# audeering/opensmile

Hardware: AMD Instinct MI355X
Metric: MFCC frames/sec (16kHz, 25ms/10ms) (higher is better)
Workload: dtype f32

## Files before the change

### opensmile_amd/csrc/lld_mfcc512.hip

```cpp
#include <hip/hip_runtime.h>
#include "kernel_timing.hpp"
#include "phase_timing.hpp"
#include "wave_lifetimes.hpp"

#include <algorithm>
#include <cmath>
#include <cstdio>
#include <cstdlib>
#include <cstring>
#include <type_traits>
#include <vector>

#include "lld_device.hpp"
#include "lld_launch.hpp"
#include "lld_params.hpp"
#include "tables.hpp"

namespace smilehip {

namespace {

constexpr int kWavesPerBlock = 8;
constexpr int kTileFrames = 32;
constexpr int kTB2Row = 65;
constexpr int kTB2Floats = 2 * (15 * kTB2Row + 3 * 16 + 16);
constexpr int kLmelFloats = 68;
constexpr int kOctetFloats = 12;
constexpr int kPbFloats = 448;
constexpr int kWaveFloats = 2080;

static_assert(kWaveFloats >= kTB2Floats && kWaveFloats >= 4 * (kLmelFloats + kPbFloats) && kWaveFloats % 4 == 0, "per-wave LDS region");
static_assert(kPbFloats % 64 == 0 && kPbFloats >= 33 * kOctetFloats, "power buffer");
static_assert(kLmelFloats >= 64 && kLmelFloats % 4 == 0 && (kLmelFloats / 4) % 2 == 1,
              "band vectors: room for the PLP vectors at +32 and +48, 16-byte aligned, neighbouring groups on different bank quads");

constexpr float C1 = 0.92387953251128673848f;
constexpr float S1 = 0.38268343236508978178f;
constexpr float R2 = 0.70710678118654752440f;

__device__ __forceinline__ void wave_lds_fence() {
  __builtin_amdgcn_fence(__ATOMIC_ACQ_REL, "wavefront");
  __builtin_amdgcn_wave_barrier();
}

__host__ __device__ constexpr int pb_pos(int k) { return k + (kOctetFloats - 8) * (k >> 3); }

__device__ __forceinline__ void dft4(float &r0, float &i0, float &r1, float &i1, float &r2, float &i2,
                                     float &r3, float &i3) {
  const float t0r = r0 + r2, t0i = i0 + i2;
  const float t1r = r0 - r2, t1i = i0 - i2;
  const float t2r = r1 + r3, t2i = i1 + i3;
  const float t3r = r1 - r3, t3i = i1 - i3;
  r0 = t0r + t2r; i0 = t0i + t2i;
  r2 = t0r - t2r; i2 = t0i - t2i;
  r1 = t1r + t3i; i1 = t1i - t3r;
  r3 = t1r - t3i; i3 = t1i + t3r;
}

__device__ __forceinline__ void cmul(float &r, float &i, float c, float s) {
  const float nr = fmaf(r, c, -i * s);
  const float ni = fmaf(r, s, i * c);
  r = nr; i = ni;
}
__device__ __forceinline__ void cmul_ns(float &r, float &i, float c, float s, float ns) {
  const float nr = fmaf(r, c, i * ns);
  const float ni = fmaf(r, s, i * c);
  r = nr; i = ni;
}

struct Dft16K {
  float c1, s1, r2, nc1, ns1, nr2;
  __device__ __forceinline__ Dft16K() : c1(C1), s1(S1), r2(R2), nc1(-C1), ns1(-S1), nr2(-R2) {
    asm volatile("" : "+s"(c1), "+s"(s1), "+s"(r2), "+s"(nc1), "+s"(ns1), "+s"(nr2));
  }
};

__device__ __forceinline__ void dft16_first(float (&re)[16], float (&im)[16], int m0) {
  dft4(re[m0], im[m0], re[m0 + 4], im[m0 + 4], re[m0 + 8], im[m0 + 8], re[m0 + 12], im[m0 + 12]);
}
__device__ __forceinline__ void dft16_twiddles(float (&re)[16], float (&im)[16], const Dft16K &K) {
  cmul_ns(re[1 + 4], im[1 + 4], K.c1, K.ns1, K.s1);
  { const float a = re[1 + 8], b = im[1 + 8]; re[1 + 8] = K.r2 * (a + b); im[1 + 8] = K.r2 * (b - a); }
  cmul_ns(re[1 + 12], im[1 + 12], K.s1, K.nc1, K.c1);
  { const float a = re[2 + 4], b = im[2 + 4]; re[2 + 4] = K.r2 * (a + b); im[2 + 4] = K.r2 * (b - a); }
  { const float a = re[2 + 8], b = im[2 + 8]; re[2 + 8] = b; im[2 + 8] = -a; }
  { const float a = re[2 + 12], b = im[2 + 12]; re[2 + 12] = K.r2 * (b - a); im[2 + 12] = K.nr2 * (a + b); }
  cmul_ns(re[3 + 4], im[3 + 4], K.s1, K.nc1, K.c1);
  { const float a = re[3 + 8], b = im[3 + 8]; re[3 + 8] = K.r2 * (b - a); im[3 + 8] = K.nr2 * (a + b); }
  cmul_ns(re[3 + 12], im[3 + 12], K.nc1, K.s1, K.ns1);
}
__device__ __forceinline__ void dft16_last(float (&re)[16], float (&im)[16], int q) {
  dft4(re[4 * q], im[4 * q], re[4 * q + 1], im[4 * q + 1], re[4 * q + 2], im[4 * q + 2], re[4 * q + 3], im[4 * q + 3]);
}
__device__ __forceinline__ void dft16_rename(float (&re)[16], float (&im)[16]) {
  float tr[16], ti[16];
#pragma unroll
  for (int q = 0; q < 4; ++q)
#pragma unroll
    for (int p = 0; p < 4; ++p) { tr[q + 4 * p] = re[4 * q + p]; ti[q + 4 * p] = im[4 * q + p]; }
#pragma unroll
  for (int k = 0; k < 16; ++k) { re[k] = tr[k]; im[k] = ti[k]; }
}
__device__ __forceinline__ void dft16(float (&re)[16], float (&im)[16], const Dft16K &K) {
#pragma unroll
  for (int m0 = 0; m0 < 4; ++m0) dft16_first(re, im, m0);
  dft16_twiddles(re, im, K);
#pragma unroll
  for (int q = 0; q < 4; ++q) dft16_last(re, im, q);
  dft16_rename(re, im);
}

template <int CTRL>
__device__ __forceinline__ float dpp_f(float v) {
  return __int_as_float(__builtin_amdgcn_update_dpp(0, __float_as_int(v), CTRL, 0xf, 0xf, true));
}

}

template <int MP, bool PLP, bool DELTA>
constexpr bool typed_loads() {
  return !PLP && !(MP == 16 && DELTA);
}
typedef float float2v __attribute__((ext_vector_type(2)));
__device__ float2v tbuffer_load_xy(__amdgpu_buffer_rsrc_t rsrc, int voffset, int soffset, int format, int aux)
    __asm("llvm.amdgcn.raw.ptr.tbuffer.load.v2f32");
__device__ float tbuffer_load_x(__amdgpu_buffer_rsrc_t rsrc, int voffset, int soffset, int format, int aux)
    __asm("llvm.amdgcn.raw.ptr.tbuffer.load.f32");
constexpr int kFmt16x2Sscaled = 5 | (3 << 4);
constexpr int kFmt16Sscaled = 2 | (3 << 4);
constexpr int kRsrcWord3 = 0x00020000, kRsrcWord3Typed = 0x00020000 | 4 | (5 << 3);

template <int MP, bool ALIGNED, bool TYPED>
struct FrameRegs {
  uint32_t v[ALIGNED && !TYPED ? MP : 2 * MP];
};

template <int MP, bool ALIGNED, bool TYPED>
__device__ __forceinline__ void pcm_prefetch(const int16_t *pcm, int64_t pcm_total, int64_t base, int H, int lane,
                                             FrameRegs<MP, ALIGNED, TYPED> &R) {
  const int64_t b0 = base < 0 ? 0 : base;
  int64_t left = (pcm_total - b0) * 2;
  left = left < 0 ? 0 : (left > 0xfffffffcLL ? 0xfffffffcLL : left);
  const __amdgpu_buffer_rsrc_t rsrc = __builtin_amdgcn_make_buffer_rsrc(const_cast<int16_t *>(pcm + b0), 0, (int)(uint32_t)left,
                                                                        TYPED ? kRsrcWord3Typed : kRsrcWord3);
  uint32_t lo = ((uint32_t)(lane >> 4) * (uint32_t)H + 2u * (uint32_t)(lane & 15)) * 2u + (uint32_t)((base - b0) * 2);
  asm volatile("" : "+v"(lo));
#pragma unroll
  for (int m = 0; m < MP; ++m) {
    if constexpr (TYPED && ALIGNED) {
      const float2v f = tbuffer_load_xy(rsrc, (int)lo + 64 * m, 0, kFmt16x2Sscaled, 0);
      R.v[2 * m] = __float_as_uint(f.x);
      R.v[2 * m + 1] = __float_as_uint(f.y);
    } else if constexpr (TYPED) {
      R.v[2 * m] = __float_as_uint(tbuffer_load_x(rsrc, (int)lo + 64 * m, 0, kFmt16Sscaled, 0));
      R.v[2 * m + 1] = __float_as_uint(tbuffer_load_x(rsrc, (int)lo + 64 * m + 2, 0, kFmt16Sscaled, 0));
    } else if constexpr (ALIGNED) {
      R.v[m] = (uint32_t)__builtin_amdgcn_raw_buffer_load_b32(rsrc, (int)lo + 64 * m, 0, 0);
    } else {
      R.v[2 * m] = (uint32_t)(int32_t)(int16_t)__builtin_amdgcn_raw_buffer_load_b16(rsrc, (int)lo + 64 * m, 0, 0);
      R.v[2 * m + 1] = (uint32_t)(int32_t)(int16_t)__builtin_amdgcn_raw_buffer_load_b16(rsrc, (int)lo + 64 * m + 2, 0, 0);
    }
  }
}

SMILEHIP_PHASE_COUNTERS(g_phase, 16, smilehip_debug_phase)
SMILEHIP_WAVE_LIFE_RECORDS(g_wave_life, smilehip_debug_wave_life)

__device__ __forceinline__ void wave_set_prio(int level) {
  switch (level & 3) {
    case 0: __builtin_amdgcn_s_setprio(0); break;
    case 1: __builtin_amdgcn_s_setprio(1); break;
    case 2: __builtin_amdgcn_s_setprio(2); break;
    default: __builtin_amdgcn_s_setprio(3); break;
  }
}

template <int MP, bool PREEMPH, bool USE_POWER, bool ALIGNED, bool PLP, int UC, bool DELTA, bool PAD0>
__device__ __forceinline__ void lld_mfcc512_body(const LldParams &P, const Fast512Tables &F) {
  extern __shared__ __attribute__((aligned(16))) float smem[];
  const int lane = threadIdx.x & 63;
  const int wave = __builtin_amdgcn_readfirstlane(threadIdx.x >> 6);
  const int g = lane >> 4;
  const int j = lane & 15;

  float2 *s_tw512 = reinterpret_cast<float2 *>(smem);
  float2 *s_win = s_tw512 + 256;
  float2 *s_tw256 = s_win + MP * 16;
  float4 *s_melw0 = reinterpret_cast<float4 *>(s_tw256 + 256);
  float4 *s_melw1 = s_melw0 + UC * 16;
  float *s_dct = reinterpret_cast<float *>(s_melw1 + UC * 16);
  float *s_plp = s_dct + 16 * 28;
  constexpr int shared_floats = 256 * 2 + MP * 16 * 2 + 256 * 2 + UC * 16 * 8 + 16 * 28 + 48;
  float *wbase = smem + shared_floats + wave * kWaveFloats;
  float *s_lmel = wbase + g * kLmelFloats;
  float *s_cep = s_lmel + 48;
  float *s_pb = wbase + 4 * kLmelFloats + g * kPbFloats;

  for (int i = threadIdx.x; i < 256; i += blockDim.x) { s_tw512[i] = F.tw512[i]; s_tw256[i] = F.tw256[i]; }
  for (int i = threadIdx.x; i < MP * 16; i += blockDim.x) s_win[i] = F.win[i];
  for (int i = threadIdx.x; i < UC * 16; i += blockDim.x) { s_melw0[i] = F.melw[2 * i]; s_melw1[i] = F.melw[2 * i + 1]; }
  for (int i = threadIdx.x; i < 16 * 28; i += blockDim.x) s_dct[i] = F.dct28[i];
  if (PLP) {
    for (int i = threadIdx.x; i < 32; i += blockDim.x) s_plp[i] = F.plp_eql[i];
    for (int i = threadIdx.x; i < 16; i += blockDim.x) s_plp[32 + i] = F.plp_sin[i];
  }
  __syncthreads();

  uint32_t mo[UC];
#pragma unroll
  for (int i = 0; i < UC; ++i) mo[i] = F.melo[i * 16 + j];
  const uint32_t lane_bands = (uint32_t)F.lane_bands[j];
  const int band0 = (int)((lane_bands >> 8) & 0xffu), band1 = (int)((lane_bands >> 16) & 0xffu);
  float uf0[UC], uf1[UC];
#pragma unroll
  for (int i = 0; i < UC; ++i) { uf0[i] = ((lane_bands >> i) & 1u) ? 1.0f : 0.0f; uf1[i] = 1.0f - uf0[i]; }
  const uint32_t out_off = (uint32_t)(g * (int)P.ld_out + j) * 4u;
  const uint32_t out_off_d = out_off + (uint32_t)P.n_mfcc * 4u;
  const uint32_t out_off_dd = out_off + (uint32_t)P.n_mfcc * 8u;
  const float nkpre = P.de ? P.k : -P.k;
  const int m0 = P.pad_left >> 5, j0 = (P.pad_left >> 1) & 15;
  float *pb_k = s_pb + pb_pos(j);
  float *pb_m = s_pb + pb_pos(256 - j);

  const Dft16K dk;
  PhaseTimer<12> PH;
  const int tile_stride = __builtin_amdgcn_readfirstlane((int)gridDim.x) * kWavesPerBlock;
  int tile = blockIdx.x * kWavesPerBlock + wave;
  const int n_tiles = DELTA ? P.n_ftiles : P.n_tiles;
  if (tile >= n_tiles) return;
  typedef typename std::conditional<DELTA, FTileRec, TileRec>::type Rec;
  typedef const __attribute__((address_space(4))) Rec *ConstRecPtr;
  const ConstRecPtr recs = DELTA ? (ConstRecPtr)(uintptr_t)P.ftile_rec : (ConstRecPtr)(uintptr_t)P.tile_rec;
  int64_t cur_samp0 = recs[tile].samp0, cur_row0 = recs[tile].row0;
  int cur_n = recs[tile].n_frames;
  int cur_live = 0, cur_e0 = 0, cur_e1 = 0, cur_lo = 0, cur_don = 0;
  if constexpr (DELTA) {
    cur_live = recs[tile].live_n; cur_e0 = recs[tile].e0; cur_e1 = recs[tile].e1; cur_lo = recs[tile].lo; cur_don = recs[tile].delta_on;
  }
  bool has_next = tile + tile_stride < n_tiles;
  int64_t nxt_samp0 = cur_samp0;
  if (has_next) nxt_samp0 = recs[tile + tile_stride].samp0;
  int tp = 0;
  constexpr bool TYPED = typed_loads<MP, PLP, DELTA>();
  FrameRegs<MP, ALIGNED, TYPED> R;
  pcm_prefetch<MP, ALIGNED, TYPED>(P.pcm, P.pcm_total, cur_samp0 - P.pad_left, P.H, lane, R);
  unsigned char *pend_row = nullptr;
  float pend_val = 0.0f;
  bool pend_live = false;
  float s_prev = 0.0f, d_cur = 0.0f;
  int b_tp = 0, b_lo = 0, b_live = 0, b_e0 = 0, b_e1 = 0, b_don = 0;
  const auto from_group = [&](int grp, float v) {
    return __int_as_float(__builtin_amdgcn_ds_bpermute(4 * ((grp << 4) | j), __float_as_int(v)));
  };
  const auto regress = [](float vm2, float vm1, float vp1, float vp2) {
    float num = 0.0f;
    num += 1.0f * (vp1 - vm1);
    num += 2.0f * (vp2 - vm2);
    return num;
  };
  const auto div10 = [](float a, bool &plain) {
    const float y = 0.1f, b = 10.0f;
    plain |= div_needs_division(a);
    return div_markstein(a, b, y);
  };
  const auto delta_fast = [&](float s_cur, float dp, float &dn, float &ddn, float &drow, bool &plain) {
    const float s1 = from_group((g + 1) & 3, g == 0 ? s_cur : s_prev);
    const float s3 = from_group((g + 3) & 3, g == 3 ? s_prev : s_cur);
    dn = div10(regress(s_prev, s1, s3, s_cur), plain);
    const float d1 = from_group((g + 1) & 3, g == 0 ? dn : dp);
    const float d3 = from_group((g + 3) & 3, g == 3 ? dp : dn);
    ddn = div10(regress(dp, d1, d3, dn), plain);
    drow = from_group((g + 2) & 3, g >= 2 ? dp : dn);
  };
  const auto delta_exact = [&](float s_cur, float dp, int btp, int lo, int live_n, float &dn, float &ddn, float &drow) {
    const auto fetch = [&](int x, int hi_c, int base, float cur, float prev) {
      x = x < lo ? lo : (x > hi_c ? hi_c : x);
      const int dd = x - base;
      const float c = from_group(dd & 3, cur), p = from_group(dd & 3, prev);
      return dd >= 0 ? c : p;
    };
    const float norm = 10.0f;
    const int fd = btp - 2 + g, fdd = btp - 4 + g, hi0 = live_n - 1, hi1 = live_n + 1;
    dn = regress(fetch(fd - 2, hi0, btp, s_cur, s_prev), fetch(fd - 1, hi0, btp, s_cur, s_prev), fetch(fd + 1, hi0, btp, s_cur, s_prev),
                 fetch(fd + 2, hi0, btp, s_cur, s_prev)) / norm;
    ddn = regress(fetch(fdd - 2, hi1, btp - 2, dn, dp), fetch(fdd - 1, hi1, btp - 2, dn, dp), fetch(fdd + 1, hi1, btp - 2, dn, dp),
                  fetch(fdd + 2, hi1, btp - 2, dn, dp)) / norm;
    drow = from_group((g + 2) & 3, g >= 2 ? dp : dn);
  };

  const int slot = (int)(__builtin_amdgcn_s_getreg((3 << 11) | 4) & 3u);
  int passes_done = 0;
  WaveLife WL;
  WL.begin();
  for (;;) {
    wave_set_prio(passes_done + slot);
    passes_done += 1;
    const bool live = tp + g < (DELTA ? cur_live : cur_n);
    PH(0);
    if constexpr (!DELTA) {
      if (pend_row != nullptr && pend_live) {
        uint32_t oo = out_off;
        asm volatile("" : "+v"(oo));
        *reinterpret_cast<float *>(pend_row + oo) = pend_val;
      }
    }
    float st_dn = 0.0f, st_ddn = 0.0f, st_drow = 0.0f;
    bool st_plain = false;
    if constexpr (DELTA) delta_fast(pend_val, d_cur, st_dn, st_ddn, st_drow, st_plain);
    float re[16], im[16];
    {
      float tprev = 0.0f;
      (void)tprev;
#pragma unroll
      for (int m = 0; m < 16; ++m) {
        if (m < MP) {
          float a, b;
          if constexpr (TYPED) {
            a = __uint_as_float(R.v[2 * m]);
            b = __uint_as_float(R.v[2 * m + 1]);
          } else if constexpr (ALIGNED) {
            a = (float)(int16_t)(R.v[m] & 0xffffu);
            b = (float)(int16_t)(R.v[m] >> 16);
          } else {
            a = (float)(int32_t)R.v[2 * m];
            b = (float)(int32_t)R.v[2 * m + 1];
          }
          float ya = a, yb = b;
          if (PREEMPH) {
            const float t = dpp_f<0x121>(b);
            const float pa = (j == 0) ? tprev : t;
            tprev = t;
            yb = fmaf(nkpre, a, b);
            ya = fmaf(nkpre, pa, a);
            if (PAD0 ? (m == 0 && j == 0) : (m == m0 && j == j0)) ya = P.one_minus_k * a;
          }
          const float2 w = s_win[m * 16 + j];
          re[m] = ya * w.x;
          im[m] = yb * w.y;
        } else {
          re[m] = 0.0f; im[m] = 0.0f;
        }
      }
    }
    PH(1);
    if constexpr (DELTA) {
      const bool clamped = !(b_tp - 6 >= b_lo && b_tp + 3 <= b_live - 1);
      if (clamped || __builtin_amdgcn_ballot_w64(st_plain && j < P.n_mfcc) != 0) delta_exact(pend_val, d_cur, b_tp, b_lo, b_live, st_dn, st_ddn, st_drow);
      const int fdd = b_tp - 4 + g;
      const bool row_live = pend_row != nullptr && j < P.n_mfcc && fdd >= b_e0 && fdd < b_e1;
      if (row_live) {
        uint32_t oo = out_off;
        asm volatile("" : "+v"(oo));
        *reinterpret_cast<float *>(pend_row + oo) = s_prev;
      }
      if (row_live && b_don) {
        uint32_t oo = out_off_d;
        asm volatile("" : "+v"(oo));
        *reinterpret_cast<float *>(pend_row + oo) = st_drow;
        oo = out_off_dd;
        asm volatile("" : "+v"(oo));
        *reinterpret_cast<float *>(pend_row + oo) = st_ddn;
      }
      s_prev = pend_val;
      d_cur = st_dn;
    }

    float2 *tbw = reinterpret_cast<float2 *>(wbase) + g * 16 + j;
    const float2 *tbr = reinterpret_cast<const float2 *>(wbase) + g * 16 + j * kTB2Row;
    {
      float2 w[4], wn[4];
#pragma unroll
      for (int p = 1; p < 4; ++p) w[p] = s_tw256[(4 * p) * 16 + j];
      w[0] = make_float2(1.0f, 0.0f);
#pragma unroll
      for (int m0 = 0; m0 < 4; ++m0) dft16_first(re, im, m0);
      dft16_twiddles(re, im, dk);
#pragma unroll
      for (int q = 0; q < 4; ++q) {
        if (q < 3) {
#pragma unroll
          for (int p = 0; p < 4; ++p) wn[p] = s_tw256[(q + 1 + 4 * p) * 16 + j];
        }
        dft16_last(re, im, q);
#pragma unroll
        for (int p = 0; p < 4; ++p) {
          const int k1 = q + 4 * p;
          if (k1 > 0) cmul(re[4 * q + p], im[4 * q + p], w[p].x, w[p].y);
          tbw[k1 * kTB2Row] = make_float2(re[4 * q + p], im[4 * q + p]);
        }
#pragma unroll
        for (int p = 0; p < 4; ++p) w[p] = wn[p];
      }
    }
    PH(3);
    {
      wave_lds_fence();
#pragma unroll
      for (int jj = 0; jj < 16; ++jj) {
        typedef const volatile __attribute__((address_space(3))) unsigned long long *LdsU64;
        const unsigned long long v = ((LdsU64)tbr)[jj];
        re[jj] = __int_as_float((int)(uint32_t)v); im[jj] = __int_as_float((int)(uint32_t)(v >> 32));
      }
      wave_lds_fence();
    }
    PH(4);
    dft16(re, im, dk);
    PH(5);

    float zr[8], zi[8];
#pragma unroll
    for (int q = 0; q < 8; ++q) {
      const float pr = q > 0 ? dpp_f<0x12f>(re[(16 - q) & 15]) : re[15];
      const float pi = q > 0 ? dpp_f<0x12f>(im[(16 - q) & 15]) : im[15];
      const float tr = __int_as_float(__builtin_amdgcn_update_dpp(__float_as_int(pr), __float_as_int(re[15 - q]), 0x101, 0xf, 0xf, false));
      const float ti = __int_as_float(__builtin_amdgcn_update_dpp(__float_as_int(pi), __float_as_int(im[15 - q]), 0x101, 0xf, 0xf, false));
      zr[q] = dpp_f<0x140>(tr);
      zi[q] = dpp_f<0x140>(ti);
    }
    float2 tw5[8];
#pragma unroll
    for (int q = 0; q < 8; ++q) tw5[q] = s_tw512[j + 16 * q];
#pragma unroll
    for (int q = 0; q < 8; ++q) {
      const float2 w = tw5[q];
      const float a = re[q], b = im[q];
      const float c = zr[q], d = zi[q];
      const float sr = a + c, si = b - d, dr = a - c, di = b + d;
      const float ur = fmaf(w.x, dr, -w.y * di);
      const float ui = fmaf(w.x, di, w.y * dr);
      const float xr = sr + ui, xi = si - ur;
      const float yr = sr - ui, yi = si + ur;
      float pk = fmaf(xi, xi, xr * xr);
      float pm = fmaf(yi, yi, yr * yr);
      if (q == 0 && j == 0) {
        const float v0 = 2.0f * (a + b), v1 = 2.0f * (a - b);
        pk = v0 * v0; pm = v1 * v1;
      }
      if (!USE_POWER) { pk = sqrtf(pk); pm = sqrtf(pm); }
      pb_k[(2 * kOctetFloats) * q] = pk;
      pb_m[-(2 * kOctetFloats) * q] = pm;
    }
    if (j == 0) {
      const float a = re[8], b = im[8];
      const float s = 4.0f * fmaf(b, b, a * a);
      s_pb[pb_pos(128)] = USE_POWER ? s : sqrtf(s);
    } else if (j < 8) {
      s_pb[pb_pos(256) + j] = 0.0f;
    }
    wave_lds_fence();

    PH(6);
    int ntp = tp + 4;
    const bool advance = ntp >= cur_n;
    const bool more = !advance || has_next;
    if (advance) ntp = 0;
    if (more)
      pcm_prefetch<MP, ALIGNED, TYPED>(P.pcm, P.pcm_total, (advance ? nxt_samp0 : cur_samp0) + (int64_t)ntp * P.H - P.pad_left, P.H, lane, R);
    else if constexpr (TYPED) {
#pragma unroll
      for (int m = 0; m < 2 * MP; ++m) R.v[m] = 0u;
    }

    PH(7);
    {
      float a0 = 0.0f, a1 = 0.0f;
#pragma unroll
      for (int i = 0; i < UC; ++i) {
        const float4 *pp = reinterpret_cast<const float4 *>(reinterpret_cast<const unsigned char *>(s_pb) + mo[i]);
        const float4 p0 = pp[0], p1 = pp[1];
        const float4 w0 = s_melw0[i * 16 + j], w1 = s_melw1[i * 16 + j];
        float acc = p0.x * w0.x;
        acc = fmaf(p0.y, w0.y, acc); acc = fmaf(p0.z, w0.z, acc); acc = fmaf(p0.w, w0.w, acc);
        acc = fmaf(p1.x, w1.x, acc); acc = fmaf(p1.y, w1.y, acc); acc = fmaf(p1.z, w1.z, acc); acc = fmaf(p1.w, w1.w, acc);
        a0 = fmaf(acc, uf0[i], a0);
        a1 = fmaf(acc, uf1[i], a1);
      }
      PH(8);
#pragma unroll
      for (int h = 0; h < 2; ++h) {
        const int b = h ? band1 : band0;
        const float acc = h ? a1 : a0;
        if (b != 0xff) {
          if (PLP) {
            float v = acc * F.mel_scale;
            v = v < P.melfloor ? P.melfloor : v;
            s_lmel[b] = __expf(P.plp_compression * __logf(v * s_plp[b]));
          } else {
            s_lmel[b] = log_mel_fast(acc * F.mel_scale, P.melfloor, P.log_floor);
          }
        }
      }
      if (j + 16 >= P.n_bands) s_lmel[j + 16] = 0.0f;
      if (j >= P.n_bands) s_lmel[j] = 0.0f;
    }
    wave_lds_fence();

    PH(9);
    if (PLP) {
      float *s_acf = s_lmel + 32;
      if (j <= P.plp_order) s_acf[j] = plp_acf_lag(s_lmel, s_dct + j * 28, P.n_bands);
      wave_lds_fence();
      if (j == 0) plp_cc_serial(s_acf, P.plp_order, s_plp + 32, s_cep);
      wave_lds_fence();
      if (j < P.n_mfcc) pend_val = s_cep[j];
    } else
    if (j < P.n_mfcc) {
      const float4 *row_c = reinterpret_cast<const float4 *>(s_dct + j * 28);
      const float4 *lm = reinterpret_cast<const float4 *>(s_lmel);
      float acc = 0.0f, dgain = 0.0f;
#pragma unroll
      for (int q = 0; q < 7; ++q) {
        const float4 l = lm[q], c = row_c[q];
        acc = fmaf(l.x, c.x, acc); acc = fmaf(l.y, c.y, acc); acc = fmaf(l.z, c.z, acc);
        if (q < 6) acc = fmaf(l.w, c.w, acc); else dgain = c.w;
      }
      pend_val = acc * dgain;
    }
    pend_live = live && j < P.n_mfcc;
    pend_row = reinterpret_cast<unsigned char *>(P.out + (cur_row0 + tp - (DELTA ? 4 : 0)) * P.ld_out);
    if constexpr (DELTA) { b_tp = tp; b_lo = cur_lo; b_live = cur_live; b_e0 = cur_e0; b_e1 = cur_e1; b_don = cur_don; }
    wave_lds_fence();
    PH(10);
    if (!more) break;
    if (advance) {
      tile += tile_stride;
      cur_samp0 = nxt_samp0; cur_row0 = recs[tile].row0; cur_n = recs[tile].n_frames;
      if constexpr (DELTA) {
        cur_live = recs[tile].live_n; cur_e0 = recs[tile].e0; cur_e1 = recs[tile].e1; cur_lo = recs[tile].lo; cur_don = recs[tile].delta_on;
      }
      has_next = tile + tile_stride < n_tiles;
      if (has_next) nxt_samp0 = recs[tile + tile_stride].samp0;
    }
    tp = ntp;
  }
  if constexpr (DELTA) {
    float dn, ddn, drow;
    delta_exact(pend_val, d_cur, b_tp, b_lo, b_live, dn, ddn, drow);
    const int fdd = b_tp - 4 + g;
    if (j < P.n_mfcc && fdd >= b_e0 && fdd < b_e1) {
      *reinterpret_cast<float *>(pend_row + out_off) = s_prev;
      if (b_don) {
        *reinterpret_cast<float *>(pend_row + out_off_d) = drow;
        *reinterpret_cast<float *>(pend_row + out_off_dd) = ddn;
      }
    }
  } else if (pend_live) {
    uint32_t oo = out_off;
    asm volatile("" : "+v"(oo));
    *reinterpret_cast<float *>(pend_row + oo) = pend_val;
  }
  PH.flush(g_phase);
  WL.end(g_wave_life, blockIdx.x, (unsigned)wave, (unsigned)passes_done);
}

template <int MP, bool PREEMPH, bool USE_POWER, bool ALIGNED, bool PLP, int UC, bool DELTA = false>
__global__ void __launch_bounds__(kWavesPerBlock * 64, 4) lld_mfcc512(LldParams P, Fast512Tables F) {
  lld_mfcc512_body<MP, PREEMPH, USE_POWER, ALIGNED, PLP, UC, DELTA, true>(P, F);
}
template <int MP, bool PREEMPH, bool USE_POWER, bool ALIGNED, bool PLP, int UC, bool DELTA = false>
__global__ void __launch_bounds__(kWavesPerBlock * 64, 4) lld_mfcc512_padded(LldParams P, Fast512Tables F) {
  lld_mfcc512_body<MP, PREEMPH, USE_POWER, ALIGNED, PLP, UC, DELTA, false>(P, F);
}

bool fast512_applicable(int Nfft, int N) { return Nfft == 512 && N <= 512 && N >= 2; }

int fast512_tile_frames() { return kTileFrames; }

int fast512_build_host(const smilehip_lld_config &cfg, const Geometry &geo, const std::vector<float> &window,
                       const MelBank &mel, const DctTables &dct, Fast512Host &h) {
  const int pad_left = cfg.zero_pad_symmetric ? (int)((geo.Nfft - geo.N) / 2) : 0;
  const int H = (int)geo.H, N = (int)geo.N;
  if (mel.n_bands > 27 || dct.n_mfcc > 16 || cfg.win_offset != 0.0 || (pad_left & 1) || (H & 1) || H < 2) return -1;
  h.mp = (pad_left + N) <= 13 * 32 ? 13 : 16;
  const char *fp = getenv("SMILEHIP_MFCC512_FORCE_PADDED");
  h.force_padded = fp != nullptr && fp[0] == '1';
  h.tw256.resize(256);
  for (int k1 = 0; k1 < 16; ++k1)
    for (int j = 0; j < 16; ++j) {
      const double a = -2.0 * M_PI * double(j * k1) / 256.0;
      h.tw256[k1 * 16 + j] = make_float2(float(cos(a)), float(sin(a)));
    }
  h.tw512.resize(256);
  for (int k = 0; k < 256; ++k) {
    const double a = -2.0 * M_PI * double(k) / 512.0;
    h.tw512[k] = make_float2(float(cos(a)), float(sin(a)));
  }
  h.win.assign(size_t(h.mp) * 16, make_float2(0.f, 0.f));
  for (int m = 0; m < h.mp; ++m)
    for (int j = 0; j < 16; ++j) {
      const int n = 2 * (j + 16 * m) - pad_left;
      float a = 0.f, b = 0.f;
      if (n >= 0 && n < N) a = float(double(window[n]) / 32767.0);
      if (n + 1 >= 0 && n + 1 < N) b = float(double(window[n + 1]) / 32767.0);
      h.win[size_t(m) * 16 + j] = make_float2(a, b);
    }
  struct Unit { int octet; float w[8]; };
  std::vector<Unit> units;
  const int nb = mel.n_bands;
  std::vector<int> first_unit(nb + 1, 0);
  for (int b = 0; b < nb; ++b) {
    int lo = -1, hi = -1;
    if (mel.rise_hi[b] > mel.rise_lo[b]) { lo = mel.rise_lo[b]; hi = mel.rise_hi[b]; }
    if (mel.fall_hi[b] > mel.fall_lo[b]) { if (lo < 0) lo = mel.fall_lo[b]; hi = mel.fall_hi[b]; }
    first_unit[b] = int(units.size());
    if (lo >= 0) {
      for (int o = lo / 8; o <= (hi - 1) / 8; ++o) {
        Unit un;
        un.octet = o;
        for (int e = 0; e < 8; ++e) {
          const int n = 8 * o + e;
          float w = 0.0f;
          if (n >= mel.rise_lo[b] && n < mel.rise_hi[b]) w = 1.0f - mel.coef[n];
          else if (n >= mel.fall_lo[b] && n < mel.fall_hi[b]) w = mel.coef[n];
          un.w[e] = w;
        }
        units.push_back(un);
      }
    }
  }
  first_unit[nb] = int(units.size());
  h.n_slots = int(units.size());
  std::vector<int> size(nb), order(nb);
  for (int b = 0; b < nb; ++b) { size[b] = first_unit[b + 1] - first_unit[b]; order[b] = b; }
  std::stable_sort(order.begin(), order.end(), [&](int x, int y) { return size[x] > size[y]; });
  int cap = 0;
  std::vector<std::pair<int, int>> lanes;
  for (int c : {6, 8}) {
    lanes.clear();
    std::vector<char> used(nb, 0);
    bool ok = true;
    for (int oi = 0; oi < nb && ok; ++oi) {
      const int a = order[oi];
      if (used[a]) continue;
      used[a] = 1;
      if (size[a] > c) { ok = false; break; }
      int partner = -1;
      for (int oj = oi + 1; oj < nb; ++oj)
        if (!used[order[oj]] && size[a] + size[order[oj]] <= c) { partner = order[oj]; break; }
      if (partner >= 0) used[partner] = 1;
      lanes.push_back({a, partner});
    }
    if (ok && (int)lanes.size() <= 16) { cap = c; break; }
  }
  if (cap == 0) return -1;
  h.mel_units = cap;
  std::vector<std::vector<int>> slot(16, std::vector<int>(cap, -1));
  for (size_t l = 0; l < lanes.size(); ++l) {
    int pos = 0;
    for (int which = 0; which < 2; ++which) {
      const int b = which ? lanes[l].second : lanes[l].first;
      if (b < 0) continue;
      for (int c = first_unit[b]; c < first_unit[b + 1]; ++c) slot[l][pos++] = c;
    }
  }
  auto step_cost = [&](int i, int &worst, int &coll) {
    int cnt[16] = {0};
    for (int l = 0; l < 16; ++l)
      if (slot[l][i] >= 0) ++cnt[units[slot[l][i]].octet & 15];
    worst = 1; coll = 0;
    for (int r = 0; r < 16; ++r) { worst = std::max(worst, cnt[r]); coll += std::max(0, cnt[r] - 1); }
  };
  auto total_cost = [&](long &primary, long &secondary) {
    primary = secondary = 0;
    for (int i = 0; i < cap; ++i) { int w, c; step_cost(i, w, c); primary += w; secondary += c; }
  };
  long best_p, best_s;
  total_cost(best_p, best_s);
  for (bool improved = true; improved;) {
    improved = false;
    for (int l = 0; l < 16; ++l)
      for (int a = 0; a < cap; ++a)
        for (int b = a + 1; b < cap; ++b) {
          if (slot[l][a] == slot[l][b]) continue;
          std::swap(slot[l][a], slot[l][b]);
          long p, s2;
          total_cost(p, s2);
          if (p < best_p || (p == best_p && s2 < best_s)) { best_p = p; best_s = s2; improved = true; }
          else std::swap(slot[l][a], slot[l][b]);
        }
  }
  h.mel_conflict_steps = int(best_p - cap);
  if (getenv("SMILEHIP_DEBUG_TABLES"))
    fprintf(stderr, "fast512: %d mel units on %zu lanes, %d per lane, bank model: %ld extra cycles over %d steps (%ld colliding lanes)\n",
            h.n_slots, lanes.size(), cap, best_p - cap, cap, best_s);
  h.melw.assign(size_t(cap) * 16 * 2, make_float4(0.f, 0.f, 0.f, 0.f));
  h.melo.assign(size_t(cap) * 16, 0u);
  h.lane_bands.assign(16, int32_t(0xffff00));
  for (int i = 0; i < cap; ++i) {
    bool taken[16] = {false};
    for (int l = 0; l < 16; ++l)
      if (slot[l][i] >= 0) taken[units[slot[l][i]].octet & 15] = true;
    for (int l = 0; l < 16; ++l) {
      const size_t idx = size_t(i) * 16 + l;
      if (slot[l][i] >= 0) {
        const Unit &un = units[slot[l][i]];
        h.melw[2 * idx] = make_float4(un.w[0], un.w[1], un.w[2], un.w[3]);
        h.melw[2 * idx + 1] = make_float4(un.w[4], un.w[5], un.w[6], un.w[7]);
        h.melo[idx] = uint32_t(un.octet) * uint32_t(kOctetFloats * 4);
      } else {
        int o = 0;
        for (int r = 0; r < 16; ++r)
          if (!taken[r]) { o = r; taken[r] = true; break; }
        h.melo[idx] = uint32_t(o) * uint32_t(kOctetFloats * 4);
      }
    }
  }
  if (getenv("SMILEHIP_DEBUG_TABLES")) {
    fprintf(stderr, "fast512: unit octets [step][lane]:");
    for (size_t idx = 0; idx < h.melo.size(); ++idx) fprintf(stderr, " %u", h.melo[idx] / uint32_t(kOctetFloats * 4));
    fprintf(stderr, "\n");
  }
  for (size_t l = 0; l < lanes.size(); ++l) {
    uint32_t mask = 0;
    const int b0 = lanes[l].first;
    for (int i = 0; i < cap; ++i)
      if (slot[l][i] >= first_unit[b0] && slot[l][i] < first_unit[b0 + 1]) mask |= 1u << i;
    h.lane_bands[l] = int32_t(mask | (uint32_t(b0) << 8) | (uint32_t(lanes[l].second < 0 ? 0xff : lanes[l].second) << 16));
  }
  h.mel_scale = mel.scale * (cfg.use_power ? 0.25f : 0.5f);
  h.dct28.assign(16 * 28, 0.0f);
  for (int r = 0; r < dct.n_mfcc; ++r)
    for (int m = 0; m < mel.n_bands; ++m) h.dct28[size_t(r) * 28 + m] = dct.cos_rows[size_t(r) * mel.n_bands + m];
  for (int r = 0; r < dct.n_mfcc; ++r) h.dct28[size_t(r) * 28 + 27] = dct.gain[r];
  return 0;
}

template <int MP, bool PREEMPH, bool USE_POWER, bool ALIGNED, bool PLP, int UC, bool DELTA = false>
static hipError_t launch_mfcc512_one(bool padded, unsigned grid, size_t lds, hipStream_t s, const LldParams &P, const Fast512Tables &F) {
  if constexpr (PREEMPH) {
    if (padded) {
      hipError_t e = hipFuncSetAttribute(reinterpret_cast<const void *>(&lld_mfcc512_padded<MP, PREEMPH, USE_POWER, ALIGNED, PLP, UC, DELTA>),
                                         hipFuncAttributeMaxDynamicSharedMemorySize, (int)lds);
      if (e != hipSuccess) return e;
      SMILEHIP_KLAUNCH((lld_mfcc512_padded<MP, PREEMPH, USE_POWER, ALIGNED, PLP, UC, DELTA>), dim3(grid), dim3(kWavesPerBlock * 64), lds, s, P, F);
      return hipSuccess;
    }
  }
  hipError_t e = hipFuncSetAttribute(reinterpret_cast<const void *>(&lld_mfcc512<MP, PREEMPH, USE_POWER, ALIGNED, PLP, UC, DELTA>),
                                     hipFuncAttributeMaxDynamicSharedMemorySize, (int)lds);
  if (e != hipSuccess) return e;
  SMILEHIP_KLAUNCH((lld_mfcc512<MP, PREEMPH, USE_POWER, ALIGNED, PLP, UC, DELTA>), dim3(grid), dim3(kWavesPerBlock * 64), lds, s, P, F);
  return hipSuccess;
}

hipError_t launch_mfcc512(const LldParams &P, const Fast512Tables &F, const Fast512Host &h, bool aligned, bool fused_delta, hipStream_t s) {
  const int shared_floats = 256 * 2 + h.mp * 16 * 2 + 256 * 2 + h.mel_units * 16 * 8 + 16 * 28 + 48;
  const size_t lds = sizeof(float) * (size_t(shared_floats) + size_t(kWavesPerBlock) * kWaveFloats);
  if (fused_delta && (!aligned || !P.ftile_rec || P.n_ftiles <= 0)) return hipErrorInvalidValue;
  unsigned grid = (unsigned)(((fused_delta ? P.n_ftiles : P.n_tiles) + kWavesPerBlock - 1) / kWavesPerBlock);
  if (grid > (unsigned)h.max_blocks) grid = (unsigned)h.max_blocks;
#ifdef SMILEHIP_DEBUG_KNOBS
  if (const char *e = getenv("SMILEHIP_DEBUG_GRID")) grid = (unsigned)atoi(e);
#endif
  bool launched = false;
  const bool padded = P.pad_left != 0 || h.force_padded;
#define SMILEHIP_LAUNCH(...)                                                                                    \
  {                                                                                                             \
    hipError_t e = launch_mfcc512_one<__VA_ARGS__>(padded, grid, lds, s, P, F);                                 \
    if (e != hipSuccess) return e;                                                                              \
    launched = true;                                                                                            \
  }
#define SMILEHIP_MATCH(MPV, PE, UP, AL, PL, UCV)                                                                \
  (!launched && h.mp == MPV && (P.preemph != 0) == PE && (P.use_power != 0) == UP && aligned == AL && (P.plp != 0) == PL && h.mel_units == UCV)
#define SMILEHIP_PICK_UD(MPV, PE, UP, PL, UCV) \
  if (fused_delta && SMILEHIP_MATCH(MPV, PE, UP, true, PL, UCV)) SMILEHIP_LAUNCH(MPV, PE, UP, true, PL, UCV, true)
#define SMILEHIP_PICK_U(MPV, PE, UP, AL, PL, UCV) \
  if (!fused_delta && SMILEHIP_MATCH(MPV, PE, UP, AL, PL, UCV)) SMILEHIP_LAUNCH(MPV, PE, UP, AL, PL, UCV)
#define SMILEHIP_PICK(MPV, PE, UP, AL, PL) SMILEHIP_PICK_U(MPV, PE, UP, AL, PL, 6) SMILEHIP_PICK_U(MPV, PE, UP, AL, PL, 8)
#define SMILEHIP_PICKD(MPV, PE, UP, PL) SMILEHIP_PICK_UD(MPV, PE, UP, PL, 6) SMILEHIP_PICK_UD(MPV, PE, UP, PL, 8)
#define SMILEHIP_PICK2(MPV, PE, UP) SMILEHIP_PICK(MPV, PE, UP, true, false) SMILEHIP_PICK(MPV, PE, UP, false, false) SMILEHIP_PICKD(MPV, PE, UP, false)
#define SMILEHIP_PICK4(MPV) SMILEHIP_PICK2(MPV, true, true) SMILEHIP_PICK2(MPV, true, false) \
                            SMILEHIP_PICK2(MPV, false, true) SMILEHIP_PICK2(MPV, false, false) \
                             \
                            SMILEHIP_PICK(MPV, true, true, true, true) SMILEHIP_PICK(MPV, true, true, false, true) \
                            SMILEHIP_PICK(MPV, false, true, true, true) SMILEHIP_PICK(MPV, false, true, false, true) \
                            SMILEHIP_PICKD(MPV, true, true, true) SMILEHIP_PICKD(MPV, false, true, true)
  SMILEHIP_PICK4(13)
  SMILEHIP_PICK4(16)
#undef SMILEHIP_PICK4
#undef SMILEHIP_PICK2
#undef SMILEHIP_PICKD
#undef SMILEHIP_PICK
#undef SMILEHIP_PICK_U
#undef SMILEHIP_PICK_UD
#undef SMILEHIP_MATCH
#undef SMILEHIP_LAUNCH
  if (!launched) return hipErrorInvalidConfiguration;
  return hipGetLastError();
}

}
```

Measured before the change: 2.975 billion.

## Permute lane-to-bin mapping so real-FFT untangle partner exchange uses one DPP hop

Remaps which frequency column each lane owns (kc permutation) so the conjugate partner needed for the real-FFT split step sits in the mirrored lane, and replaces the multi-DPP shuffle (row_ror, row_shl, row_bcast per element) with a single row_mirror DPP move plus a masked fixup under a hand-set exec mask. LDS read addresses, twiddle indices and power-bin store positions are all remapped to match. This removes several cross-lane ops per value, at the cost of inline asm that overrides the exec mask and a lane permutation that must stay consistent across stages.

```diff
diff --git a/opensmile_amd/csrc/lld_mfcc512.hip b/opensmile_amd/csrc/lld_mfcc512.hip
--- a/opensmile_amd/csrc/lld_mfcc512.hip
+++ b/opensmile_amd/csrc/lld_mfcc512.hip
@@ -115,10 +115,56 @@
   return __int_as_float(__builtin_amdgcn_update_dpp(0, __float_as_int(v), CTRL, 0xf, 0xf, true));
 }
 
+__device__ __forceinline__ void untangle_partner(float (&x)[16], float (&y)[16]) {
+  unsigned long long sv;
+  asm volatile(
+      "s_mov_b64 %[sv], exec\n"
+      "s_mov_b32 exec_lo, 0x7ffe7ffe\n"
+      "s_mov_b32 exec_hi, 0x7ffe7ffe\n"
+      "v_mov_b32_dpp %[x8], %[x8] row_mirror row_mask:0xf bank_mask:0xf\n"
+      "v_mov_b32_dpp %[x9], %[x9] row_mirror row_mask:0xf bank_mask:0xf\n"
+      "v_mov_b32_dpp %[x10], %[x10] row_mirror row_mask:0xf bank_mask:0xf\n"
+      "v_mov_b32_dpp %[x11], %[x11] row_mirror row_mask:0xf bank_mask:0xf\n"
+      "v_mov_b32_dpp %[x12], %[x12] row_mirror row_mask:0xf bank_mask:0xf\n"
+      "v_mov_b32_dpp %[x13], %[x13] row_mirror row_mask:0xf bank_mask:0xf\n"
+      "v_mov_b32_dpp %[x14], %[x14] row_mirror row_mask:0xf bank_mask:0xf\n"
+      "v_mov_b32_dpp %[x15], %[x15] row_mirror row_mask:0xf bank_mask:0xf\n"
+      "v_mov_b32_dpp %[y8], %[y8] row_mirror row_mask:0xf bank_mask:0xf\n"
+      "v_mov_b32_dpp %[y9], %[y9] row_mirror row_mask:0xf bank_mask:0xf\n"
+      "v_mov_b32_dpp %[y10], %[y10] row_mirror row_mask:0xf bank_mask:0xf\n"
+      "v_mov_b32_dpp %[y11], %[y11] row_mirror row_mask:0xf bank_mask:0xf\n"
+      "v_mov_b32_dpp %[y12], %[y12] row_mirror row_mask:0xf bank_mask:0xf\n"
+      "v_mov_b32_dpp %[y13], %[y13] row_mirror row_mask:0xf bank_mask:0xf\n"
+      "v_mov_b32_dpp %[y14], %[y14] row_mirror row_mask:0xf bank_mask:0xf\n"
+      "v_mov_b32_dpp %[y15], %[y15] row_mirror row_mask:0xf bank_mask:0xf\n"
+      "s_mov_b32 exec_lo, 0x00010001\n"
+      "s_mov_b32 exec_hi, 0x00010001\n"
+      "v_mov_b32 %[x8], %[x9]\n"
+      "v_mov_b32 %[x9], %[x10]\n"
+      "v_mov_b32 %[x10], %[x11]\n"
+      "v_mov_b32 %[x11], %[x12]\n"
+      "v_mov_b32 %[x12], %[x13]\n"
+      "v_mov_b32 %[x13], %[x14]\n"
+      "v_mov_b32 %[x14], %[x15]\n"
+      "v_mov_b32 %[y8], %[y9]\n"
+      "v_mov_b32 %[y9], %[y10]\n"
+      "v_mov_b32 %[y10], %[y11]\n"
+      "v_mov_b32 %[y11], %[y12]\n"
+      "v_mov_b32 %[y12], %[y13]\n"
+      "v_mov_b32 %[y13], %[y14]\n"
+      "v_mov_b32 %[y14], %[y15]\n"
+      "s_mov_b64 exec, %[sv]\n"
+      : [sv] "=&s"(sv), [x8] "+v"(x[8]), [x9] "+v"(x[9]), [x10] "+v"(x[10]), [x11] "+v"(x[11]), [x12] "+v"(x[12]), [x13] "+v"(x[13]), [x14] "+v"(x[14]), [x15] "+v"(x[15]), [y8] "+v"(y[8]), [y9] "+v"(y[9]), [y10] "+v"(y[10]), [y11] "+v"(y[11]), [y12] "+v"(y[12]), [y13] "+v"(y[13]), [y14] "+v"(y[14]), [y15] "+v"(y[15]));
+}
+
 }
 
 template <int MP, bool PLP, bool DELTA>
 constexpr bool typed_loads() {
+  return !PLP && !(MP == 16 && DELTA);
+}
+template <int MP, bool PLP, bool DELTA>
+constexpr bool one_hop_exchange() {
   return !PLP && !(MP == 16 && DELTA);
 }
 typedef float float2v __attribute__((ext_vector_type(2)));
@@ -219,8 +265,10 @@
   const uint32_t out_off_dd = out_off + (uint32_t)P.n_mfcc * 8u;
   const float nkpre = P.de ? P.k : -P.k;
   const int m0 = P.pad_left >> 5, j0 = (P.pad_left >> 1) & 15;
-  float *pb_k = s_pb + pb_pos(j);
-  float *pb_m = s_pb + pb_pos(256 - j);
+  constexpr bool kOneHop = one_hop_exchange<MP, PLP, DELTA>();
+  const int kc = !kOneHop ? j : (j < 8 ? j : (j == 15 ? 8 : j + 1));
+  float *pb_k = s_pb + pb_pos(kc);
+  float *pb_m = s_pb + pb_pos(256 - kc);
 
   const Dft16K dk;
   PhaseTimer<12> PH;
@@ -366,7 +414,7 @@
     }
 
     float2 *tbw = reinterpret_cast<float2 *>(wbase) + g * 16 + j;
-    const float2 *tbr = reinterpret_cast<const float2 *>(wbase) + g * 16 + j * kTB2Row;
+    const float2 *tbr = reinterpret_cast<const float2 *>(wbase) + g * 16 + kc * kTB2Row;
     {
       float2 w[4], wn[4];
 #pragma unroll
@@ -407,24 +455,35 @@
     dft16(re, im, dk);
     PH(5);
 
-    float zr[8], zi[8];
-#pragma unroll
-    for (int q = 0; q < 8; ++q) {
-      const float pr = q > 0 ? dpp_f<0x12f>(re[(16 - q) & 15]) : re[15];
-      const float pi = q > 0 ? dpp_f<0x12f>(im[(16 - q) & 15]) : im[15];
-      const float tr = __int_as_float(__builtin_amdgcn_update_dpp(__float_as_int(pr), __float_as_int(re[15 - q]), 0x101, 0xf, 0xf, false));
-      const float ti = __int_as_float(__builtin_amdgcn_update_dpp(__float_as_int(pi), __float_as_int(im[15 - q]), 0x101, 0xf, 0xf, false));
-      zr[q] = dpp_f<0x140>(tr);
-      zi[q] = dpp_f<0x140>(ti);
+    float p128 = 0.0f;
+    if constexpr (kOneHop) {
+      const float a = re[8], b = im[8];
+      p128 = 4.0f * fmaf(b, b, a * a);
+      untangle_partner(re, im);
+    } else {
+      float zr[8], zi[8];
+#pragma unroll
+      for (int q = 0; q < 8; ++q) {
+        const float pr = q > 0 ? dpp_f<0x12f>(re[(16 - q) & 15]) : re[15];
+        const float pi = q > 0 ? dpp_f<0x12f>(im[(16 - q) & 15]) : im[15];
+        const float tr = __int_as_float(__builtin_amdgcn_update_dpp(__float_as_int(pr), __float_as_int(re[15 - q]), 0x101, 0xf, 0xf, false));
+        const float ti = __int_as_float(__builtin_amdgcn_update_dpp(__float_as_int(pi), __float_as_int(im[15 - q]), 0x101, 0xf, 0xf, false));
+        zr[q] = dpp_f<0x140>(tr);
+        zi[q] = dpp_f<0x140>(ti);
+      }
+      const float a = re[8], b = im[8];
+      p128 = 4.0f * fmaf(b, b, a * a);
+#pragma unroll
+      for (int q = 0; q < 8; ++q) { re[15 - q] = zr[q]; im[15 - q] = zi[q]; }
     }
     float2 tw5[8];
 #pragma unroll
-    for (int q = 0; q < 8; ++q) tw5[q] = s_tw512[j + 16 * q];
+    for (int q = 0; q < 8; ++q) tw5[q] = s_tw512[kc + 16 * q];
 #pragma unroll
     for (int q = 0; q < 8; ++q) {
       const float2 w = tw5[q];
       const float a = re[q], b = im[q];
-      const float c = zr[q], d = zi[q];
+      const float c = re[15 - q], d = im[15 - q];
       const float sr = a + c, si = b - d, dr = a - c, di = b + d;
       const float ur = fmaf(w.x, dr, -w.y * di);
       const float ui = fmaf(w.x, di, w.y * dr);
@@ -441,9 +500,7 @@
       pb_m[-(2 * kOctetFloats) * q] = pm;
     }
     if (j == 0) {
-      const float a = re[8], b = im[8];
-      const float s = 4.0f * fmaf(b, b, a * a);
-      s_pb[pb_pos(128)] = USE_POWER ? s : sqrtf(s);
+      s_pb[pb_pos(128)] = USE_POWER ? p128 : sqrtf(p128);
     } else if (j < 8) {
       s_pb[pb_pos(256) + j] = 0.0f;
     }
```

Result: faster. 3.040 billion (median of 6 runs) (+2.2%).
